# rdd0582/mri_superresolution

Hardware: AMD Instinct MI355X
Metric: 2D MRI slices/sec (train fwd+bwd) 256×256 U-Net; PSNR/SSIM vs ref (higher is better)
Workload: dtype bf16; 1 GPU; UNetSuperRes base_filters=64 depth=4, 256x256 slices -> 512x512, batch=16/GPU bf16, L1+SSIM(0.4), train step fwd+bwd+Adam+SSIM metric; global_batch=16, parallelism=dp1

## Files before the change

include/mrisr.h:

```cpp
#ifndef MRISR_H
#define MRISR_H

#include <stddef.h>
#include <stdint.h>

#ifdef __cplusplus
extern "C" {
#endif

#define MRISR_OK 0
#define MRISR_E_ARG (-1)
#define MRISR_E_SHAPE (-2)
#define MRISR_E_DTYPE (-3)
#define MRISR_E_HIP (-4)
#define MRISR_E_UNSUPPORTED (-5)

#define MRISR_F32 0
#define MRISR_BF16 1
#define MRISR_F16 2

#define MRISR_SRC_RAW 0
#define MRISR_SRC_NORM 1
#define MRISR_SRC_RELU 2
#define MRISR_SP_NONE 0
// ... 164 lines not shown
int mrisr_head_backward(int dtype, const void* x, const float* scale, const float* shift,
                        const float* w, const float* out, const float* dout, void* da, float* dw,
                        float* db, int N, int H, int W, int C, void* stream);
int mrisr_head_forward_multi(int dtype, const void* x, const float* scale, const float* shift,
                             const float* w, const float* b, float* out, int N, int H, int W, int C,
                             int K, void* stream);
int mrisr_head_backward_multi(int dtype, const void* x, const float* scale, const float* shift,
                              const float* w, const float* out, const float* dout, void* da,
                              float* dw, float* db, int N, int H, int W, int C, int K, void* stream);

int mrisr_ssim_l1_forward(const float* a, const float* b, double* sums, float* coef, int N, int H,
                          int W, float val_range, float sigma, void* stream);
int mrisr_ssim_l1_backward(const float* a, const float* b, const float* coef, const double* sums,
                           const float* gscale, float l1_w, float ssim_w, float* da, int N, int H,
                           int W, float sigma, void* stream);
int mrisr_ssim_l1_forward_win(const float* a, const float* b, double* sums, float* coef, int N, int H, int W,
                              float val_range, float sigma, int window_size, void* stream);
int mrisr_ssim_l1_backward_win(const float* a, const float* b, const float* coef, const double* sums,
                               const float* gscale, float l1_w, float ssim_w, float* da, int N, int H, int W,
                               float sigma, int window_size, void* stream);

int mrisr_loss_finalize(const double* sums, int N, int H, int W, float l1_w, float ssim_w, float* out,
                        void* stream);

int mrisr_image_metrics(const float* a, const float* b, double* sums, int N, int H, int W, float val_range, float sigma,
                        int window_size, void* stream);
int mrisr_metrics_finalize(const double* sums, int N, int H, int W, float val_range, double* out, void* stream);

int mrisr_vgg_input_channels(void);
int mrisr_vgg_input_forward(int dtype, const float* x, void* out, size_t npix, void* stream);
int mrisr_vgg_input_backward(int dtype, const void* dx3, const float* gscale, float scale, float* dimg,
                             size_t npix, void* stream);
int mrisr_maxpool2_forward(int dtype, const void* x, void* out, int N, int H, int W, int C, void* stream);
int mrisr_maxpool2_backward(int dtype, const void* x, const void* dy, void* dx, int N, int H, int W, int C,
                            int relu_gate, void* stream);
int mrisr_feature_loss(int dtype, const void* a, const void* b, size_t n, int kind, double* sum16, float* out,
                       void* da, int relu_gate, void* stream);

int mrisr_adam_step(float* p, const float* g, float* m, float* v, size_t n, float lr, float beta1,
                    float beta2, float eps, float weight_decay, int step, float grad_scale,
                    void* stream);
int mrisr_adam_step_amp(float* p, const float* g, float* m, float* v, size_t n, float lr, float beta1, float beta2,
                        float eps, float weight_decay, int* step_device, float grad_mul,
                        const float* loss_scale_device, const float* found_inf_device, void* stream);

int mrisr_u8_histogram(const uint8_t* img, size_t pixels_per_image, int batch, unsigned* hist, void* stream);
// ... 157 lines not shown
```

mri_superresolution_amd/_lib.py:

```python
from __future__ import annotations

import ctypes as C
import os

from .tuning import TUNING

_HERE = os.path.dirname(os.path.abspath(__file__))
LIB_PATH = TUNING.lib_path or os.path.join(_HERE, "libmrisr.so")

F32, BF16, F16 = 0, 1, 2
SRC_RAW, SRC_NORM, SRC_RELU = 0, 1, 2
SP_NONE, SP_POOL2, SP_UP2, SP_HEAD = 0, 1, 2, 3
COMBINE_CONCAT, COMBINE_BLEND = 0, 1
OUT_PLAIN, OUT_PIXEL_SHUFFLE2 = 0, 1
UP2_BILINEAR, UP2_BICUBIC, UP2_SHARP_BILINEAR = 0, 1, 2
WINDOW_F32, WINDOW_I16 = 0, 1
VOLBLEND_SET, VOLBLEND_ADD, VOLBLEND_FINISH = 0, 1, 2
MORPH_DILATE, MORPH_ERODE = 0, 1
RESAMPLE_LINEAR, RESAMPLE_CUBIC, RESAMPLE_AREA, RESAMPLE_LANCZOS4 = 1, 2, 3, 4
BIAS_PAIR, BIAS_HUM, BIAS_LOWPASS = 0, 1, 2
RESAMPLE_NEAREST = 5
PACK_RING = 256
PACK_UPADJ = 512
STAT_SLOTS = 16
# ... 79 lines not shown
    "mrisr_act_bwd_apply_fused": (_i, [_i, _vp, _fp, _fp, _i, C.POINTER(Consumer), _fp, _fp, C.POINTER(GnBwdFin), _vp, _i, _i,
                                       _i, _i, _vp]),
    "mrisr_act_bwd_onepass_slots": (_i, []),
    "mrisr_act_bwd_onepass_barrier_words": (_i, []),
    "mrisr_act_bwd_onepass_ok": (_i, [_i, _i, C.POINTER(Consumer), _i, _i, _i, _i]),
    "mrisr_act_bwd_onepass": (_i, [_i, _vp, _fp, _fp, _fp, _i, C.POINTER(Consumer), _fp, _vp, C.POINTER(GnBwdFin), _vp, _i, _i, _i,
                                   _i, _vp]),
    "mrisr_act_bwd_apply_fused_unshuffle": (_i, [_i, _vp, _fp, _fp, C.POINTER(Consumer), _fp, C.POINTER(GnBwdFin), _vp, _fp, _i,
                                                 _i, _i, _i, _vp]),
    "mrisr_act_bwd_blend_ok": (_i, [_i, _i, _i, _i, _i]),
    "mrisr_act_bwd_blend_reduce": (_i, [_i, _vp, C.POINTER(BlendBranch), C.POINTER(BlendBranch), _fp, _i, _i, _i, _i, _i, _vp]),
    "mrisr_act_bwd_blend_apply": (_i, [_i, _vp, C.POINTER(BlendBranch), C.POINTER(BlendBranch), _fp, C.POINTER(GnBwdFin),
                                       C.POINTER(GnBwdFin), _vp, _vp, _fp, _i, _i, _i, _i, _vp]),
    "mrisr_channel_sum": (_i, [_i, _vp, _fp, _sz, _i, _vp]),
    "mrisr_head_forward": (_i, [_i, _vp, _fp, _fp, _fp, _fp, _fp, _i, _i, _i, _i, _vp]),
    "mrisr_head_backward": (_i, [_i, _vp, _fp, _fp, _fp, _fp, _fp, _vp, _fp, _fp, _i, _i, _i, _i, _vp]),
    "mrisr_head_forward_multi": (_i, [_i, _vp, _fp, _fp, _fp, _fp, _fp, _i, _i, _i, _i, _i, _vp]),
    "mrisr_head_backward_multi": (_i, [_i, _vp, _fp, _fp, _fp, _fp, _fp, _vp, _fp, _fp, _i, _i, _i, _i, _i, _vp]),
    "mrisr_ssim_l1_forward": (_i, [_fp, _fp, _dp, _fp, _i, _i, _i, _f, _f, _vp]),
    "mrisr_ssim_l1_backward": (_i, [_fp, _fp, _fp, _dp, _fp, _f, _f, _fp, _i, _i, _i, _f, _vp]),
    "mrisr_ssim_l1_forward_win": (_i, [_fp, _fp, _dp, _fp, _i, _i, _i, _f, _f, _i, _vp]),
    "mrisr_ssim_l1_backward_win": (_i, [_fp, _fp, _fp, _dp, _fp, _f, _f, _fp, _i, _i, _i, _f, _i, _vp]),
    "mrisr_loss_finalize": (_i, [_dp, _i, _i, _i, _f, _f, _fp, _vp]),
    "mrisr_image_metrics": (_i, [_fp, _fp, _dp, _i, _i, _i, _f, _f, _i, _vp]),
    "mrisr_metrics_finalize": (_i, [_dp, _i, _i, _i, _f, _dp, _vp]),
    "mrisr_vgg_input_channels": (_i, []),
    "mrisr_vgg_input_forward": (_i, [_i, _fp, _vp, _sz, _vp]),
    "mrisr_vgg_input_backward": (_i, [_i, _vp, _fp, _f, _fp, _sz, _vp]),
    "mrisr_maxpool2_forward": (_i, [_i, _vp, _vp, _i, _i, _i, _i, _vp]),
    "mrisr_maxpool2_backward": (_i, [_i, _vp, _vp, _vp, _i, _i, _i, _i, _i, _vp]),
    "mrisr_feature_loss": (_i, [_i, _vp, _vp, _sz, _i, _dp, _fp, _vp, _i, _vp]),
    "mrisr_adam_step": (_i, [_fp, _fp, _fp, _fp, _sz, _f, _f, _f, _f, _f, _i, _f, _vp]),
    "mrisr_adam_step_amp": (_i, [_fp, _fp, _fp, _fp, _sz, _f, _f, _f, _f, _f, _vp, _f, _fp, _fp, _vp]),
    "mrisr_u8_histogram": (_i, [_vp, _sz, _i, _vp, _vp]),
    "mrisr_u8_percentile_normalise": (_i, [_vp, _vp, _sz, _i, _d, _d, _fp, _fp, _vp]),
    "mrisr_f32_to_u8": (_i, [_fp, _vp, _sz, _vp]),
    "mrisr_u8_upscale2": (_i, [_vp, _vp, _fp, _i, _i, _i, _i, _vp]),
    "mrisr_u8_to_unit_f32": (_i, [_vp, _fp, _sz, _vp]),
    "mrisr_augment_geo_u8": (_i, [_vp, _vp, _i, _i, _i, _vp, _dp, _vp]),
    "mrisr_augment_finish_u8": (_i, [_vp, _fp, _i, _sz, _vp, _dp, _vp]),
    "mrisr_lowfield_dirichlet": (_i, [_i, _d, _fp, _fp]),
    "mrisr_lowfield_workspace_bytes": (_sz, [_i, _i, _i]),
    "mrisr_lowfield_simulate": (_i, [_vp, _i, _i, _i, _d, _fp, _fp, _fp, _fp, _f, _fp, _fp, _vp, _vp, _vp, _fp, _vp]),
    "mrisr_lowfield_dirichlet_any": (_i, [_i, _d, _fp, _fp]),
    "mrisr_lowfield_simulate_f32": (_i, [_fp, _i, _i, _i, _d, _fp, _fp, _fp, _fp, _f, _fp, _fp, _vp, _vp, _fp, _vp]),
    "mrisr_resample_taps": (_i, [_i, _i, _i, _i, _vp, _vp, _fp]),
# ... 26 lines not shown
    "mrisr_f32_masked_percentiles_workspace_bytes": (_sz, [_i]),
    "mrisr_f32_volume_masked_percentiles": (_i, [_fp, _vp, _sz, C.POINTER(C.c_double), _i, _fp, _vp, _vp, _vp]),
    "mrisr_f32_volume_piecewise_map": (_i, [_fp, _sz, _fp, _fp, _i, _fp, _vp]),
    "mrisr_f32_volume_smooth_masked": (_i, [_fp, _vp, _vp, _i, _i, _i, _fp, _i, _fp, _i, _fp, _i, _fp, _fp, _fp, _vp]),
    "mrisr_f32_volume_bias_apply": (_i, [_fp, _sz, _fp, _fp, _fp, _fp, _fp, _vp, _f, _i, _fp, _fp, _vp]),
    "mrisr_f32_volume_nlm": (_i, [_fp, _i, _i, _i, _i, _i, _fp, _fp, _fp, _vp]),
    "mrisr_f32_volume_noise_workspace_bytes": (_sz, []),
    "mrisr_f32_volume_noise_params": (_i, [_fp, _vp, _sz, _f, _f, _fp, _vp, _vp, _vp]),
    "mrisr_f32_volume_deform_workspace_bytes": (_sz, []),
    "mrisr_f32_volume_warp": (_i, [_fp, _fp, _i, _i, _i, _i, _f, _fp, _vp]),
    "mrisr_f32_volume_demons_force": (_i, [_fp, _fp, _fp, _i, _i, _i, _f, _f, _fp, _vp, _vp, _vp]),
    "mrisr_f32_volume_field_smooth": (_i, [_fp, _fp, _i, _i, _i, _i, _fp, _i, _vp, _vp, _vp]),
    "mrisr_f32_volume_jacobian_stats": (_i, [_fp, _i, _i, _i, _fp, _vp, _vp, _vp]),
    "mrisr_f32_volume_field_compose": (_i, [_fp, _fp, _i, _i, _i, _fp, _vp]),
    "mrisr_f32_volume_demons_update": (_i, [_fp, _fp, _fp, _i, _i, _i, _f, _f, _f, _fp, _vp, _vp, _vp]),
    "mrisr_f32_volume_warp_matrix": (_i, [_fp, _i, _i, _i, _fp, _i, _i, _i, C.POINTER(C.c_double), _i, _f, _fp, _vp]),
    "mrisr_f32_volume_quantise": (_i, [_fp, _vp, _sz, _fp, _vp, _vp, _vp, _vp, _vp]),
    "mrisr_u8_volume_joint_hist": (_i, [_vp, _vp, _sz, _i, _vp, _vp]),
    "mrisr_u8_volume_icm_half": (_i, [_vp, _vp, _i, _i, _i, _i, _vp, _i, _i, _vp, _vp]),
    "mrisr_u8_volume_confusion": (_i, [_vp, _vp, _vp, _sz, _i, _vp, _vp]),
}

_lib = None
ABI_VERSION = 323


def load():
    global _lib
    if _lib is not None:
        return _lib
    if not os.path.exists(LIB_PATH):
        raise RuntimeError(
            f"{LIB_PATH} not found: the HIP kernel library is not built. Run "
            "`python -m mri_superresolution_amd.build` (needs hipcc); there is no CPU fallback.")
    lib = C.CDLL(LIB_PATH)
    missing = [name for name in SIGNATURES if not hasattr(lib, name)]
    if missing:
        raise RuntimeError(f"{LIB_PATH} lacks {len(missing)} symbol(s) of include/mrisr.h ({', '.join(missing[:4])}...): "
                           "header/library drift - rebuild with `python -m mri_superresolution_amd.build`")
    for name, (res, args) in SIGNATURES.items():
        fn = getattr(lib, name)
        fn.restype = res
        fn.argtypes = args
    if int(lib.mrisr_version()) != ABI_VERSION:
        raise RuntimeError(f"{LIB_PATH} is version {int(lib.mrisr_version())}, these bindings need {ABI_VERSION} (struct layouts "
                           "changed): rebuild with `python -m mri_superresolution_amd.build`")
    global STAT_SLOTS
# ... 48 lines not shown
```

mri_superresolution_amd/csrc/api.cpp:

```cpp
#include "common.h"
thread_local char g_mrisr_err[512] = "";
extern "C" const char* mrisr_last_error(void) { return g_mrisr_err; }
extern "C" int mrisr_version(void) { return 323; }
extern "C" int mrisr_stat_slots(void) { return MRISR_STAT_SLOTS; }
```

mri_superresolution_amd/csrc/loss.hip:

```cpp
#include "common.h"

constexpr int kMaxWin = 15;
constexpr int kTW = 32, kTH = 8;

struct GaussWin { float g[kMaxWin]; };

static GaussWin make_window(float sigma, int win) {
    GaussWin w;
    float sum = 0.f;
    for (int i = 0; i < kMaxWin; ++i) w.g[i] = 0.f;
    for (int i = 0; i < win; ++i) {
        const float c = (float)(i - win / 2);
        w.g[i] = expf(-(c * c) / (2.0f * sigma * sigma));
        sum += w.g[i];
    }
    for (int i = 0; i < win; ++i) w.g[i] /= sum;
    return w;
}

constexpr int kFT = 32;
template <int kWin, bool kSq = false>
__global__ __launch_bounds__(256) void ssim_l1_fwd_kernel(const float* __restrict__ a, const float* __restrict__ b,
                                                          double* __restrict__ sums, float* __restrict__ coef, int N,
                                                          int H, int W, float c1, float c2, const GaussWin win) {
    constexpr int kHalo = kWin / 2, kFL = kFT + 2 * kHalo;
    __shared__ float ta[kFL][kFL + 2], tb[kFL][kFL + 2];
    __shared__ float hz[5][kFL][kFT + 1];
    constexpr int kSums = kSq ? 3 : 2;
    __shared__ float part[4][kSums];
    const int t = threadIdx.x, n = blockIdx.z;
    const int x0 = blockIdx.x * kFT, y0 = blockIdx.y * kFT;
    const float* an = a + (size_t)n * H * W;
    const float* bn = b + (size_t)n * H * W;
    for (int i = t; i < kFL * kFL; i += 256) {
        const int ly = i / kFL, lx = i - ly * kFL;
        const int gy = y0 + ly - kHalo, gx = x0 + lx - kHalo;
        const bool in = gy >= 0 && gy < H && gx >= 0 && gx < W;
        ta[ly][lx] = in ? an[(size_t)gy * W + gx] : 0.f;
        tb[ly][lx] = in ? bn[(size_t)gy * W + gx] : 0.f;
    }
    __syncthreads();
    for (int sgm = t; sgm < kFL * (kFT / 4); sgm += 256) {
        const int ly = sgm / (kFT / 4), lx = (sgm - ly * (kFT / 4)) * 4;
        float u[kWin + 3], v[kWin + 3];
#pragma unroll
        for (int k = 0; k < kWin + 3; ++k) { u[k] = ta[ly][lx + k]; v[k] = tb[ly][lx + k]; }
#pragma unroll
        for (int o = 0; o < 4; ++o) {
            float s0 = 0.f, s1 = 0.f, s2 = 0.f, s3 = 0.f, s4 = 0.f;
#pragma unroll
            for (int k = 0; k < kWin; ++k) {
                const float uu = u[o + k], vv = v[o + k], g = win.g[k];
                s0 += g * uu; s1 += g * vv; s2 += g * uu * uu; s3 += g * vv * vv; s4 += g * uu * vv;
            }
            hz[0][ly][lx + o] = s0; hz[1][ly][lx + o] = s1; hz[2][ly][lx + o] = s2; hz[3][ly][lx + o] = s3; hz[4][ly][lx + o] = s4;
        }
    }
    __syncthreads();
    const int lx = t & (kFT - 1), ly0 = (t >> 5) * 4;
    float m[4][5];
#pragma unroll
    for (int o = 0; o < 4; ++o)
#pragma unroll
        for (int q = 0; q < 5; ++q) m[o][q] = 0.f;
#pragma unroll
    for (int q = 0; q < 5; ++q) {
        float col[kWin + 3];
#pragma unroll
        for (int k = 0; k < kWin + 3; ++k) col[k] = hz[q][ly0 + k][lx];
#pragma unroll
        for (int o = 0; o < 4; ++o)
#pragma unroll
            for (int k = 0; k < kWin; ++k) m[o][q] += win.g[k] * col[o + k];
    }
    float l1 = 0.f, sv = 0.f, sq = 0.f;
    const int gx = x0 + lx;
#pragma unroll
    for (int o = 0; o < 4; ++o) {
        const int gy = y0 + ly0 + o;
        if (gy < H && gx < W) {
            const float mu1 = m[o][0], mu2 = m[o][1];
            const float mu1sq = mu1 * mu1, mu2sq = mu2 * mu2, mu12 = mu1 * mu2;
            const float s11 = m[o][2] - mu1sq, s22 = m[o][3] - mu2sq, s12 = m[o][4] - mu12;
            const float A1 = 2.f * mu12 + c1, A2 = 2.f * s12 + c2, B1 = mu1sq + mu2sq + c1, B2 = s11 + s22 + c2;
            const float inv = 1.f / (B1 * B2);
            const float S = A1 * A2 * inv;
            sv += S;
            const float d = ta[ly0 + o + kHalo][lx + kHalo] - tb[ly0 + o + kHalo][lx + kHalo];
            l1 += fabsf(d);
            if (kSq) sq += d * d;
            if (coef) {
                const size_t plane = (size_t)N * H * W, oo = ((size_t)n * H + gy) * W + gx;
                coef[oo] = 2.f * mu2 * (A2 - A1) * inv - 2.f * mu1 * S / B1 + 2.f * mu1 * S / B2;
                coef[plane + oo] = -S / B2;
                coef[2 * plane + oo] = 2.f * A1 * inv;
            }
        }
    }
    l1 = wave_sum(l1);
    sv = wave_sum(sv);
    if (kSq) sq = wave_sum(sq);
    if ((t & 63) == 0) {
        part[t >> 6][0] = l1; part[t >> 6][1] = sv;
        if (kSq) part[t >> 6][kSums - 1] = sq;
    }
    __syncthreads();
    if (t < kSums) atomic_add_f64(&sums[(size_t)n * kSums + t], (double)(part[0][t] + part[1][t] + part[2][t] + part[3][t]));
}

template <int WIN>
static void launch_ssim_fwd(dim3 grid, hipStream_t s, const float* a, const float* b, double* sums, float* coef, int N, int H, int W,
                            float c1, float c2, float sigma) {
    ssim_l1_fwd_kernel<WIN><<<grid, 256, 0, s>>>(a, b, sums, coef, N, H, W, c1, c2, make_window(sigma, WIN));
}
#define MRISR_SSIM_WIN_SWITCH(win, CALL) \
    switch (win) { case 3: CALL(3); break; case 5: CALL(5); break; case 7: CALL(7); break; case 9: CALL(9); break; \
                   case 11: CALL(11); break; case 13: CALL(13); break; default: CALL(15); break; }

extern "C" int mrisr_ssim_l1_forward_win(const float* a, const float* b, double* sums, float* coef, int N, int H, int W,
                                         float val_range, float sigma, int window_size, void* stream) {
    if (!a || !b || !sums) MRISR_FAIL(MRISR_E_ARG, "ssim_l1_forward: null pointer");
    if (N <= 0 || H <= 0 || W <= 0 || N > 65535) MRISR_FAIL(MRISR_E_SHAPE, "ssim_l1_forward: N%d H%d W%d", N, H, W);
    if (window_size < 3 || window_size > kMaxWin || !(window_size & 1)) MRISR_FAIL(MRISR_E_UNSUPPORTED, "ssim_l1_forward: window_size %d (odd, 3..15)", window_size);
    const float c1 = (0.01f * val_range) * (0.01f * val_range), c2 = (0.03f * val_range) * (0.03f * val_range);
    dim3 grid(ceil_div(W, kFT), ceil_div(H, kFT), N);
    hipStream_t s = (hipStream_t)stream;
#define MRISR_CALL(WIN) launch_ssim_fwd<WIN>(grid, s, a, b, sums, coef, N, H, W, c1, c2, sigma)
    MRISR_SSIM_WIN_SWITCH(window_size, MRISR_CALL)
#undef MRISR_CALL
    MRISR_CHECK_LAUNCH("ssim_l1_forward");
    return MRISR_OK;
}
extern "C" int mrisr_ssim_l1_forward(const float* a, const float* b, double* sums, float* coef, int N, int H, int W,
                                     float val_range, float sigma, void* stream) {
    return mrisr_ssim_l1_forward_win(a, b, sums, coef, N, H, W, val_range, sigma, 11, stream);
}

template <int WIN>
static void launch_metrics(dim3 grid, hipStream_t s, const float* a, const float* b, double* sums, int N, int H, int W,
                           float c1, float c2, float sigma) {
    ssim_l1_fwd_kernel<WIN, true><<<grid, 256, 0, s>>>(a, b, sums, nullptr, N, H, W, c1, c2, make_window(sigma, WIN));
}
extern "C" int mrisr_image_metrics(const float* a, const float* b, double* sums, int N, int H, int W, float val_range,
                                   float sigma, int window_size, void* stream) {
    if (!a || !b || !sums) MRISR_FAIL(MRISR_E_ARG, "image_metrics: null pointer");
    if (N <= 0 || H <= 0 || W <= 0 || N > 65535) MRISR_FAIL(MRISR_E_SHAPE, "image_metrics: N%d H%d W%d", N, H, W);
    if (window_size < 3 || window_size > kMaxWin || !(window_size & 1)) MRISR_FAIL(MRISR_E_UNSUPPORTED, "image_metrics: window_size %d (odd, 3..15)", window_size);
    const float c1 = (0.01f * val_range) * (0.01f * val_range), c2 = (0.03f * val_range) * (0.03f * val_range);
    dim3 grid(ceil_div(W, kFT), ceil_div(H, kFT), N);
    hipStream_t s = (hipStream_t)stream;
#define MRISR_CALL(WIN) launch_metrics<WIN>(grid, s, a, b, sums, N, H, W, c1, c2, sigma)
    MRISR_SSIM_WIN_SWITCH(window_size, MRISR_CALL)
#undef MRISR_CALL
    MRISR_CHECK_LAUNCH("image_metrics");
    return MRISR_OK;
}

__global__ __launch_bounds__(64) void metrics_finalize_kernel(const double* __restrict__ sums, int N, double inv_pixels, double range2,
                                                              double* __restrict__ out) {
    const int n = blockIdx.x * 64 + threadIdx.x;
    if (n >= N) return;
    const double mae = sums[3 * n] * inv_pixels, ssim = sums[3 * n + 1] * inv_pixels, mse = sums[3 * n + 2] * inv_pixels;
    out[5 * n] = ssim;
    out[5 * n + 1] = mse;
    out[5 * n + 2] = __dsqrt_rn(mse);
    out[5 * n + 3] = mae;
    out[5 * n + 4] = mse < 1e-10 ? 100.0 : 10.0 * log10(range2 / mse);
}

extern "C" int mrisr_metrics_finalize(const double* sums, int N, int H, int W, float val_range, double* out, void* stream) {
    if (!sums || !out) MRISR_FAIL(MRISR_E_ARG, "metrics_finalize: null pointer");
    if (N <= 0 || H <= 0 || W <= 0) MRISR_FAIL(MRISR_E_SHAPE, "metrics_finalize: N%d H%d W%d", N, H, W);
    metrics_finalize_kernel<<<ceil_div(N, 64), 64, 0, (hipStream_t)stream>>>(sums, N, 1.0 / ((double)H * W), (double)val_range * (double)val_range, out);
    MRISR_CHECK_LAUNCH("metrics_finalize");
    return MRISR_OK;
}

template <int kWin>
__global__ __launch_bounds__(256) void ssim_l1_bwd_kernel(const float* __restrict__ a, const float* __restrict__ b,
                                                          const float* __restrict__ coef, const double* __restrict__ sums,
                                                          const float* __restrict__ gscale, float l1_w, float ssim_w,
                                                          float* __restrict__ da, int N, int H, int W, const GaussWin win) {
    constexpr int kHalo = kWin / 2, kLW = kTW + 2 * kHalo, kLH = kTH + 2 * kHalo;
    __shared__ float tc[3][kLH][kLW + 1];
    __shared__ float hz[3][kLH][kTW + 1];
    const int t = threadIdx.x, n = blockIdx.z;
    const int x0 = blockIdx.x * kTW, y0 = blockIdx.y * kTH;
    const size_t plane = (size_t)N * H * W;
    const float gs = gscale ? gscale[0] : 1.f;
    const double numel = (double)N * H * W;
    float sw = 0.f;
    if (ssim_w != 0.f) {
        if (sums) {
            double tot = 0.0;
            for (int i = 0; i < N; ++i) tot += sums[(size_t)i * 2 + 1];
            const double mean = tot / numel;
            if (mean >= 0.0 && mean <= 1.0) sw = ssim_w;
        } else {
            sw = ssim_w;
        }
    }
    if (sw != 0.f) {
        for (int i = t; i < kLH * kLW; i += 256) {
            const int ly = i / kLW, lx = i - ly * kLW;
            const int gy = y0 + ly - kHalo, gx = x0 + lx - kHalo;
            const bool in = gy >= 0 && gy < H && gx >= 0 && gx < W;
            const size_t o = ((size_t)n * H + gy) * W + gx;
#pragma unroll
            for (int q = 0; q < 3; ++q) tc[q][ly][lx] = in ? coef[q * plane + o] : 0.f;
        }
        __syncthreads();
        for (int i = t; i < kLH * kTW; i += 256) {
            const int ly = i / kTW, lx = i - ly * kTW;
            float s[3] = {0.f, 0.f, 0.f};
#pragma unroll
            for (int k = 0; k < kWin; ++k)
#pragma unroll
                for (int q = 0; q < 3; ++q) s[q] += win.g[k] * tc[q][ly][lx + k];
#pragma unroll
            for (int q = 0; q < 3; ++q) hz[q][ly][lx] = s[q];
        }
        __syncthreads();
    }
    const int ly = t / kTW, lx = t - ly * kTW;
    const int gy = y0 + ly, gx = x0 + lx;
    if (gy < H && gx < W) {
        const size_t o = ((size_t)n * H + gy) * W + gx;
        const float av = a[o], bv = b[o];
        float g = 0.f;
        if (l1_w != 0.f) {
            const float d = av - bv;
            g += l1_w * (d > 0.f ? 1.f : (d < 0.f ? -1.f : 0.f));
        }
        if (sw != 0.f) {
            float m[3] = {0.f, 0.f, 0.f};
#pragma unroll
            for (int k = 0; k < kWin; ++k)
#pragma unroll
                for (int q = 0; q < 3; ++q) m[q] += win.g[k] * hz[q][ly + k][lx];
            g -= sw * (m[0] + 2.f * av * m[1] + bv * m[2]);
        }
        da[o] = gs * g * (float)(1.0 / numel);
    }
}

template <int WIN>
static void launch_ssim_bwd(dim3 grid, hipStream_t s, const float* a, const float* b, const float* coef, const double* sums,
                            const float* gscale, float l1_w, float ssim_w, float* da, int N, int H, int W, float sigma) {
    ssim_l1_bwd_kernel<WIN><<<grid, 256, 0, s>>>(a, b, coef, sums, gscale, l1_w, ssim_w, da, N, H, W, make_window(sigma, WIN));
}
extern "C" int mrisr_ssim_l1_backward_win(const float* a, const float* b, const float* coef, const double* sums,
                                          const float* gscale, float l1_w, float ssim_w, float* da, int N, int H, int W,
                                          float sigma, int window_size, void* stream) {
    if (!a || !b || !da) MRISR_FAIL(MRISR_E_ARG, "ssim_l1_backward: null pointer");
    if (ssim_w != 0.f && !coef) MRISR_FAIL(MRISR_E_ARG, "ssim_l1_backward: ssim term needs coef");
    if (N <= 0 || H <= 0 || W <= 0 || N > 65535) MRISR_FAIL(MRISR_E_SHAPE, "ssim_l1_backward: N%d H%d W%d", N, H, W);
    if (window_size < 3 || window_size > kMaxWin || !(window_size & 1)) MRISR_FAIL(MRISR_E_UNSUPPORTED, "ssim_l1_backward: window_size %d (odd, 3..15)", window_size);
    dim3 grid(ceil_div(W, kTW), ceil_div(H, kTH), N);
    hipStream_t s = (hipStream_t)stream;
#define MRISR_CALL(WIN) launch_ssim_bwd<WIN>(grid, s, a, b, coef, sums, gscale, l1_w, ssim_w, da, N, H, W, sigma)
    MRISR_SSIM_WIN_SWITCH(window_size, MRISR_CALL)
#undef MRISR_CALL
    MRISR_CHECK_LAUNCH("ssim_l1_backward");
    return MRISR_OK;
}
extern "C" int mrisr_ssim_l1_backward(const float* a, const float* b, const float* coef, const double* sums,
                                      const float* gscale, float l1_w, float ssim_w, float* da, int N, int H, int W,
                                      float sigma, void* stream) {
    return mrisr_ssim_l1_backward_win(a, b, coef, sums, gscale, l1_w, ssim_w, da, N, H, W, sigma, 11, stream);
}

__global__ void loss_finalize_kernel(const double* __restrict__ sums, int N, double inv_numel, double inv_per_sample,
                                     float l1_w, float ssim_w, float* __restrict__ out) {
    if (threadIdx.x != 0 || blockIdx.x != 0) return;
    double l1 = 0.0, ss = 0.0;
    for (int i = 0; i < N; ++i) {
        l1 += sums[2 * i];
        ss += sums[2 * i + 1];
        out[3 + i] = (float)(sums[2 * i + 1] * inv_per_sample);
    }
    const float l1m = (float)(l1 * inv_numel), sm = (float)(ss * inv_numel);
    float total = 0.f;
    if (l1_w > 0.f) total += l1_w * l1m;
    if (ssim_w > 0.f) total += ssim_w * (1.f - fminf(fmaxf(sm, 0.f), 1.f));
    out[0] = total;
    out[1] = l1m;
    out[2] = sm;
}

extern "C" int mrisr_loss_finalize(const double* sums, int N, int H, int W, float l1_w, float ssim_w, float* out,
                                   void* stream) {
    if (!sums || !out) MRISR_FAIL(MRISR_E_ARG, "loss_finalize: null pointer");
    loss_finalize_kernel<<<1, 64, 0, (hipStream_t)stream>>>(sums, N, 1.0 / ((double)N * H * W), 1.0 / ((double)H * W), l1_w, ssim_w, out);
    MRISR_CHECK_LAUNCH("loss_finalize");
    return MRISR_OK;
}
```

mri_superresolution_amd/utils/losses.py:

```python
from __future__ import annotations

import torch
import torch.nn as nn

from .. import _lib as L

VGG_MEAN = [0.485, 0.456, 0.406]
VGG_STD = [0.229, 0.224, 0.225]

_WINDOW = 11


def gaussian_window(window_size: int, sigma: float):
    coords = torch.arange(window_size, dtype=torch.float32) - window_size // 2
    g = torch.exp(-(coords ** 2) / (2 * sigma ** 2))
    return g / g.sum()


def create_window(window_size: int, channel: int, sigma: float, device: torch.device):
    w1 = gaussian_window(window_size, sigma).to(device).unsqueeze(1)
    return w1.mm(w1.t()).expand(channel, 1, window_size, window_size).contiguous()


def _planes(t: torch.Tensor) -> torch.Tensor:
# ... 11 lines not shown
def _sums_key(a, b, sigma, val_range, win):
    return (a.data_ptr(), a._version, tuple(a.shape), b.data_ptr(), b._version, float(sigma), float(val_range), int(win),
            L.inplace_epoch, torch.cuda.current_stream().cuda_stream)


def _check_window(window_size):
    if not isinstance(window_size, int) or window_size < 3 or window_size > 15 or window_size % 2 == 0:
        raise NotImplementedError(f"the fused SSIM kernel supports odd window sizes 3..15, got {window_size!r}")


class _SSIML1(torch.autograd.Function):

    @staticmethod
    def forward(ctx, img1, img2, l1_w, ssim_w, sigma, val_range, kind, holder, track, win=_WINDOW, track2=False):
        a, b = _planes(img1), _planes(img2)
        if a.shape != b.shape:
            raise ValueError(f"shape mismatch {tuple(a.shape)} vs {tuple(b.shape)}")
        n, c, h, w = a.shape
        planes = n * c
        need_grad = bool(track)
        st = L.stream_ptr()
        global _last_sums
        key = _sums_key(a, b, sigma, val_range, win)
        if not need_grad and not track2 and _last_sums is not None and _last_sums[0] == key:
            sums, coef = _last_sums[1], None
        else:
            sums = torch.zeros(planes * 2, dtype=torch.float64, device=a.device)
            coef = torch.empty(3 * planes * h * w, dtype=torch.float32, device=a.device) if (need_grad and ssim_w != 0) else None
            L.call("mrisr_ssim_l1_forward_win", a.data_ptr(), b.data_ptr(), sums.data_ptr(), L.ptr(coef), planes, h, w,
                   float(val_range), float(sigma), int(win), st, nbytes=planes * h * w * (8 + (12 if coef is not None else 0)))
            _last_sums = (key, sums, a, b)
        comp = torch.empty(3 + planes, dtype=torch.float32, device=a.device)
        L.call("mrisr_loss_finalize", sums.data_ptr(), planes, h, w, float(l1_w), float(ssim_w), comp.data_ptr(), st)
        if holder is not None:
            holder.last_components = comp
        ctx.save_for_backward(a, b, coef, sums)
        ctx.cfg = (float(l1_w), float(ssim_w), float(sigma), kind, planes, h, w, int(win), float(val_range), bool(track), bool(track2))
        return comp[0].clone() if kind == 0 else comp[2].clone()

    @staticmethod
    def backward(ctx, gout):
        a, b, coef, sums = ctx.saved_tensors
        l1_w, ssim_w, sigma, kind, planes, h, w, win, val_range, track, track2 = ctx.cfg
        g = gout.detach().to(torch.float32).reshape(1).contiguous()
        st = L.stream_ptr()

        def grad_first(x, y, cf):
            dx = torch.empty_like(x)
            if kind == 0:
                L.call("mrisr_ssim_l1_backward_win", x.data_ptr(), y.data_ptr(), L.ptr(cf), sums.data_ptr(), g.data_ptr(),
                       l1_w, ssim_w, dx.data_ptr(), planes, h, w, sigma, win, st,
                       nbytes=planes * h * w * (12 + (12 if cf is not None else 0)))
            else:
                L.call("mrisr_ssim_l1_backward_win", x.data_ptr(), y.data_ptr(), L.ptr(cf), None, g.data_ptr(),
                       0.0, -1.0, dx.data_ptr(), planes, h, w, sigma, win, st)
            return dx

        da = grad_first(a, b, coef) if track else None
        db = None
        if track2:
            coef2 = None
            if ssim_w != 0:
                coef2 = torch.empty(3 * planes * h * w, dtype=torch.float32, device=a.device)
                scratch = torch.zeros(planes * 2, dtype=torch.float64, device=a.device)
                L.call("mrisr_ssim_l1_forward_win", b.data_ptr(), a.data_ptr(), scratch.data_ptr(), coef2.data_ptr(), planes, h, w,
                       val_range, sigma, win, st)
            db = grad_first(b, a, coef2)
        return da, db, None, None, None, None, None, None, None, None, None


def ssim(img1, img2, window_size=11, sigma=1.5, val_range=1.0, device=None, window=None, size_average=True):
    _check_window(window_size)
    holder = type("H", (), {})()
    grads = torch.is_grad_enabled()
    val = _SSIML1.apply(img1, img2, 0.0, 1.0, sigma, val_range, 1, holder, grads and img1.requires_grad, window_size,
                        grads and img2.requires_grad)
    if size_average:
        result = val
    else:
        n, c = img1.shape[0], img1.shape[1]
        result = holder.last_components[3:].view(n, c).mean(1)
    if img1.dtype != torch.float32 and img1.dtype == img2.dtype:
        result = result.to(img1.dtype)
    return result


class VGGFeatureExtractor(nn.Module):

# ... 112 lines not shown
```

Measured before the change: 2113 slices/s.

## Restructure SSIM+L1 loss kernels: vectorized tile loads, per-tile slots, fused finalize

The SSIM/L1 forward kernel now loads its halo tile with float4 pieces into registers before writing shared memory. Each block writes its partial sums to a per-tile slot instead of doing a double atomicAdd, and a single finalize kernel reduces the slots and writes the scalar return value. This removes the zero-fill memset, the float64 atomics and the clone kernel. The backward kernel moves to the same 32x32 tiles with 4 outputs per thread, vectorized coef loads and a wave-parallel gate reduction. The SSIM loss is a small part of a full U-Net train step, and the change adds slot buffer allocations and more shared memory per block.

Measured after the change: 2128 slices/s (median of 6 runs). No clear change (+0.7%).

```diff
diff --git a/include/mrisr.h b/include/mrisr.h
--- a/include/mrisr.h
+++ b/include/mrisr.h
@@ -210,6 +210,11 @@
 
 int mrisr_loss_finalize(const double* sums, int N, int H, int W, float l1_w, float ssim_w, float* out,
                         void* stream);
+int mrisr_ssim_l1_tiles(int H, int W);
+int mrisr_ssim_l1_forward_slots(const float* a, const float* b, double* slots, float* coef, int N, int H, int W,
+                                float val_range, float sigma, int window_size, void* stream);
+int mrisr_loss_finalize_slots(const double* slots, double* sums, int N, int H, int W, float l1_w, float ssim_w, float* out,
+                              float* ret, int kind, void* stream);
 
 int mrisr_image_metrics(const float* a, const float* b, double* sums, int N, int H, int W, float val_range, float sigma,
                         int window_size, void* stream);
diff --git a/mri_superresolution_amd/_lib.py b/mri_superresolution_amd/_lib.py
--- a/mri_superresolution_amd/_lib.py
+++ b/mri_superresolution_amd/_lib.py
@@ -125,6 +125,9 @@
     "mrisr_ssim_l1_forward_win": (_i, [_fp, _fp, _dp, _fp, _i, _i, _i, _f, _f, _i, _vp]),
     "mrisr_ssim_l1_backward_win": (_i, [_fp, _fp, _fp, _dp, _fp, _f, _f, _fp, _i, _i, _i, _f, _i, _vp]),
     "mrisr_loss_finalize": (_i, [_dp, _i, _i, _i, _f, _f, _fp, _vp]),
+    "mrisr_ssim_l1_tiles": (_i, [_i, _i]),
+    "mrisr_ssim_l1_forward_slots": (_i, [_fp, _fp, _dp, _fp, _i, _i, _i, _f, _f, _i, _vp]),
+    "mrisr_loss_finalize_slots": (_i, [_dp, _dp, _i, _i, _i, _f, _f, _fp, _fp, _i, _vp]),
     "mrisr_image_metrics": (_i, [_fp, _fp, _dp, _i, _i, _i, _f, _f, _i, _vp]),
     "mrisr_metrics_finalize": (_i, [_dp, _i, _i, _i, _f, _dp, _vp]),
     "mrisr_vgg_input_channels": (_i, []),
@@ -197,7 +200,7 @@
 }
 
 _lib = None
-ABI_VERSION = 323
+ABI_VERSION = 324
 
 
 def load():
diff --git a/mri_superresolution_amd/csrc/api.cpp b/mri_superresolution_amd/csrc/api.cpp
--- a/mri_superresolution_amd/csrc/api.cpp
+++ b/mri_superresolution_amd/csrc/api.cpp
@@ -1,5 +1,5 @@
 #include "common.h"
 thread_local char g_mrisr_err[512] = "";
 extern "C" const char* mrisr_last_error(void) { return g_mrisr_err; }
-extern "C" int mrisr_version(void) { return 323; }
+extern "C" int mrisr_version(void) { return 324; }
 extern "C" int mrisr_stat_slots(void) { return MRISR_STAT_SLOTS; }
diff --git a/mri_superresolution_amd/csrc/loss.hip b/mri_superresolution_amd/csrc/loss.hip
--- a/mri_superresolution_amd/csrc/loss.hip
+++ b/mri_superresolution_amd/csrc/loss.hip
@@ -1,7 +1,6 @@
 #include "common.h"
 
 constexpr int kMaxWin = 15;
-constexpr int kTW = 32, kTH = 8;
 
 struct GaussWin { float g[kMaxWin]; };
 
@@ -19,42 +18,94 @@
 }
 
 constexpr int kFT = 32;
+constexpr int kApron = 8;
+constexpr int kSW = kFT + 2 * kApron;
+constexpr int kSS = kSW + 1;
+constexpr int kHS = kFT + 1;
+
+static inline int ssim_tiles(int H, int W) { return ceil_div(W, kFT) * ceil_div(H, kFT); }
+
+__device__ __forceinline__ float4 load_piece(const float* __restrict__ p, int gy, int gx, int H, int W, bool vec) {
+    const bool row_in = gy >= 0 && gy < H;
+    const float* row = p + (size_t)min(max(gy, 0), H - 1) * W;
+    float4 v;
+    if (vec) {
+        v = *reinterpret_cast<const float4*>(row + min(max(gx, 0), W - 4));
+        if (!(row_in && gx >= 0 && gx < W)) v = make_float4(0.f, 0.f, 0.f, 0.f);
+    } else {
+        v.x = row[min(max(gx, 0), W - 1)];
+        v.y = row[min(max(gx + 1, 0), W - 1)];
+        v.z = row[min(max(gx + 2, 0), W - 1)];
+        v.w = row[min(max(gx + 3, 0), W - 1)];
+        if (!(row_in && gx >= 0 && gx < W)) v.x = 0.f;
+        if (!(row_in && gx + 1 >= 0 && gx + 1 < W)) v.y = 0.f;
+        if (!(row_in && gx + 2 >= 0 && gx + 2 < W)) v.z = 0.f;
+        if (!(row_in && gx + 3 >= 0 && gx + 3 < W)) v.w = 0.f;
+    }
+    return v;
+}
+__device__ __forceinline__ void store_piece(float* __restrict__ row, float4 v) {
+    row[0] = v.x; row[1] = v.y; row[2] = v.z; row[3] = v.w;
+}
+#define MRISR_PIECE(i, ly, lc)            \
+    const int pq_ = (i) / (kSW / 4);      \
+    const int lc = ((i) - pq_ * (kSW / 4)) * 4, ly = min(pq_, kFL - 1)
+
+template <int kWin, int kOut, int kPlane>
+__device__ __forceinline__ void ssim_fwd_hblur(const float* __restrict__ pa, const float* __restrict__ pb, float* __restrict__ ph,
+                                               const GaussWin& win) {
+    float u[kWin + kOut - 1], v[kWin + kOut - 1];
+#pragma unroll
+    for (int k = 0; k < kWin + kOut - 1; ++k) { u[k] = pa[k]; v[k] = pb[k]; }
+#pragma unroll
+    for (int o = 0; o < kOut; ++o) {
+        float s0 = 0.f, s1 = 0.f, s2 = 0.f, s3 = 0.f, s4 = 0.f;
+#pragma unroll
+        for (int k = 0; k < kWin; ++k) {
+            const float uu = u[o + k], vv = v[o + k], g = win.g[k];
+            s0 += g * uu; s1 += g * vv; s2 += g * uu * uu; s3 += g * vv * vv; s4 += g * uu * vv;
+        }
+        ph[o] = s0; ph[kPlane + o] = s1; ph[2 * kPlane + o] = s2; ph[3 * kPlane + o] = s3; ph[4 * kPlane + o] = s4;
+    }
+}
+
 template <int kWin, bool kSq = false>
 __global__ __launch_bounds__(256) void ssim_l1_fwd_kernel(const float* __restrict__ a, const float* __restrict__ b,
-                                                          double* __restrict__ sums, float* __restrict__ coef, int N,
-                                                          int H, int W, float c1, float c2, const GaussWin win) {
+                                                          double* __restrict__ sums, double* __restrict__ slots,
+                                                          float* __restrict__ coef, int N, int H, int W, float c1, float c2,
+                                                          const GaussWin win) {
     constexpr int kHalo = kWin / 2, kFL = kFT + 2 * kHalo;
-    __shared__ float ta[kFL][kFL + 2], tb[kFL][kFL + 2];
-    __shared__ float hz[5][kFL][kFT + 1];
+    constexpr int kOff = kApron - kHalo;
+    constexpr int kPieces = kFL * (kSW / 4), kRounds = (kPieces + 255) / 256;
+    __shared__ float ta[kFL][kSS], tb[kFL][kSS];
+    __shared__ float hz[5][kFL][kHS];
     constexpr int kSums = kSq ? 3 : 2;
     __shared__ float part[4][kSums];
     const int t = threadIdx.x, n = blockIdx.z;
     const int x0 = blockIdx.x * kFT, y0 = blockIdx.y * kFT;
     const float* an = a + (size_t)n * H * W;
     const float* bn = b + (size_t)n * H * W;
-    for (int i = t; i < kFL * kFL; i += 256) {
-        const int ly = i / kFL, lx = i - ly * kFL;
-        const int gy = y0 + ly - kHalo, gx = x0 + lx - kHalo;
-        const bool in = gy >= 0 && gy < H && gx >= 0 && gx < W;
-        ta[ly][lx] = in ? an[(size_t)gy * W + gx] : 0.f;
-        tb[ly][lx] = in ? bn[(size_t)gy * W + gx] : 0.f;
+    const bool vec = (W & 3) == 0 && (((uintptr_t)a | (uintptr_t)b) & 15) == 0;
+    float4 ra[kRounds], rb[kRounds];
+#pragma unroll
+    for (int r = 0; r < kRounds; ++r) {
+        MRISR_PIECE(t + r * 256, ly, lc);
+        ra[r] = load_piece(an, y0 + ly - kHalo, x0 - kApron + lc, H, W, vec);
+        rb[r] = load_piece(bn, y0 + ly - kHalo, x0 - kApron + lc, H, W, vec);
+    }
+#pragma unroll
+    for (int r = 0; r < kRounds; ++r) {
+        MRISR_PIECE(t + r * 256, ly, lc);
+        if (t + r * 256 < kPieces) { store_piece(&ta[ly][lc], ra[r]); store_piece(&tb[ly][lc], rb[r]); }
     }
     __syncthreads();
-    for (int sgm = t; sgm < kFL * (kFT / 4); sgm += 256) {
-        const int ly = sgm / (kFT / 4), lx = (sgm - ly * (kFT / 4)) * 4;
-        float u[kWin + 3], v[kWin + 3];
-#pragma unroll
-        for (int k = 0; k < kWin + 3; ++k) { u[k] = ta[ly][lx + k]; v[k] = tb[ly][lx + k]; }
-#pragma unroll
-        for (int o = 0; o < 4; ++o) {
-            float s0 = 0.f, s1 = 0.f, s2 = 0.f, s3 = 0.f, s4 = 0.f;
-#pragma unroll
-            for (int k = 0; k < kWin; ++k) {
-                const float uu = u[o + k], vv = v[o + k], g = win.g[k];
-                s0 += g * uu; s1 += g * vv; s2 += g * uu * uu; s3 += g * vv * vv; s4 += g * uu * vv;
-            }
-            hz[0][ly][lx + o] = s0; hz[1][ly][lx + o] = s1; hz[2][ly][lx + o] = s2; hz[3][ly][lx + o] = s3; hz[4][ly][lx + o] = s4;
-        }
+    {
+        const int ly = t >> 3, lx = (t & 7) * 4;
+        ssim_fwd_hblur<kWin, 4, kFL * kHS>(&ta[ly][lx + kOff], &tb[ly][lx + kOff], &hz[0][ly][lx], win);
+    }
+    if (t < (kFL - 32) * (kFT / 2)) {
+        const int ly = 32 + (t >> 4), lx = (t & 15) * 2;
+        ssim_fwd_hblur<kWin, 2, kFL * kHS>(&ta[ly][lx + kOff], &tb[ly][lx + kOff], &hz[0][ly][lx], win);
     }
     __syncthreads();
     const int lx = t & (kFT - 1), ly0 = (t >> 5) * 4;
@@ -86,7 +137,7 @@
             const float inv = 1.f / (B1 * B2);
             const float S = A1 * A2 * inv;
             sv += S;
-            const float d = ta[ly0 + o + kHalo][lx + kHalo] - tb[ly0 + o + kHalo][lx + kHalo];
+            const float d = ta[ly0 + o + kHalo][lx + kApron] - tb[ly0 + o + kHalo][lx + kApron];
             l1 += fabsf(d);
             if (kSq) sq += d * d;
             if (coef) {
@@ -105,41 +156,58 @@
         if (kSq) part[t >> 6][kSums - 1] = sq;
     }
     __syncthreads();
-    if (t < kSums) atomic_add_f64(&sums[(size_t)n * kSums + t], (double)(part[0][t] + part[1][t] + part[2][t] + part[3][t]));
+    if (t < kSums) {
+        const double v = (double)(part[0][t] + part[1][t] + part[2][t] + part[3][t]);
+        if (slots) {
+            const size_t tile = (size_t)blockIdx.y * gridDim.x + blockIdx.x, tiles = (size_t)gridDim.x * gridDim.y;
+            slots[((size_t)n * tiles + tile) * kSums + t] = v;
+        } else {
+            atomic_add_f64(&sums[(size_t)n * kSums + t], v);
+        }
+    }
 }
 
 template <int WIN>
-static void launch_ssim_fwd(dim3 grid, hipStream_t s, const float* a, const float* b, double* sums, float* coef, int N, int H, int W,
-                            float c1, float c2, float sigma) {
-    ssim_l1_fwd_kernel<WIN><<<grid, 256, 0, s>>>(a, b, sums, coef, N, H, W, c1, c2, make_window(sigma, WIN));
+static void launch_ssim_fwd(dim3 grid, hipStream_t s, const float* a, const float* b, double* sums, double* slots, float* coef, int N,
+                            int H, int W, float c1, float c2, float sigma) {
+    ssim_l1_fwd_kernel<WIN><<<grid, 256, 0, s>>>(a, b, sums, slots, coef, N, H, W, c1, c2, make_window(sigma, WIN));
 }
 #define MRISR_SSIM_WIN_SWITCH(win, CALL) \
     switch (win) { case 3: CALL(3); break; case 5: CALL(5); break; case 7: CALL(7); break; case 9: CALL(9); break; \
                    case 11: CALL(11); break; case 13: CALL(13); break; default: CALL(15); break; }
 
-extern "C" int mrisr_ssim_l1_forward_win(const float* a, const float* b, double* sums, float* coef, int N, int H, int W,
-                                         float val_range, float sigma, int window_size, void* stream) {
-    if (!a || !b || !sums) MRISR_FAIL(MRISR_E_ARG, "ssim_l1_forward: null pointer");
+static int ssim_l1_forward(const float* a, const float* b, double* sums, double* slots, float* coef, int N, int H, int W,
+                           float val_range, float sigma, int window_size, void* stream) {
+    if (!a || !b || (!sums && !slots)) MRISR_FAIL(MRISR_E_ARG, "ssim_l1_forward: null pointer");
     if (N <= 0 || H <= 0 || W <= 0 || N > 65535) MRISR_FAIL(MRISR_E_SHAPE, "ssim_l1_forward: N%d H%d W%d", N, H, W);
     if (window_size < 3 || window_size > kMaxWin || !(window_size & 1)) MRISR_FAIL(MRISR_E_UNSUPPORTED, "ssim_l1_forward: window_size %d (odd, 3..15)", window_size);
     const float c1 = (0.01f * val_range) * (0.01f * val_range), c2 = (0.03f * val_range) * (0.03f * val_range);
     dim3 grid(ceil_div(W, kFT), ceil_div(H, kFT), N);
     hipStream_t s = (hipStream_t)stream;
-#define MRISR_CALL(WIN) launch_ssim_fwd<WIN>(grid, s, a, b, sums, coef, N, H, W, c1, c2, sigma)
+#define MRISR_CALL(WIN) launch_ssim_fwd<WIN>(grid, s, a, b, sums, slots, coef, N, H, W, c1, c2, sigma)
     MRISR_SSIM_WIN_SWITCH(window_size, MRISR_CALL)
 #undef MRISR_CALL
     MRISR_CHECK_LAUNCH("ssim_l1_forward");
     return MRISR_OK;
 }
+extern "C" int mrisr_ssim_l1_forward_win(const float* a, const float* b, double* sums, float* coef, int N, int H, int W,
+                                         float val_range, float sigma, int window_size, void* stream) {
+    return ssim_l1_forward(a, b, sums, nullptr, coef, N, H, W, val_range, sigma, window_size, stream);
+}
 extern "C" int mrisr_ssim_l1_forward(const float* a, const float* b, double* sums, float* coef, int N, int H, int W,
                                      float val_range, float sigma, void* stream) {
     return mrisr_ssim_l1_forward_win(a, b, sums, coef, N, H, W, val_range, sigma, 11, stream);
 }
+extern "C" int mrisr_ssim_l1_tiles(int H, int W) { return H > 0 && W > 0 ? ssim_tiles(H, W) : 0; }
+extern "C" int mrisr_ssim_l1_forward_slots(const float* a, const float* b, double* slots, float* coef, int N, int H, int W,
+                                           float val_range, float sigma, int window_size, void* stream) {
+    return ssim_l1_forward(a, b, nullptr, slots, coef, N, H, W, val_range, sigma, window_size, stream);
+}
 
 template <int WIN>
 static void launch_metrics(dim3 grid, hipStream_t s, const float* a, const float* b, double* sums, int N, int H, int W,
                            float c1, float c2, float sigma) {
-    ssim_l1_fwd_kernel<WIN, true><<<grid, 256, 0, s>>>(a, b, sums, nullptr, N, H, W, c1, c2, make_window(sigma, WIN));
+    ssim_l1_fwd_kernel<WIN, true><<<grid, 256, 0, s>>>(a, b, sums, nullptr, nullptr, N, H, W, c1, c2, make_window(sigma, WIN));
 }
 extern "C" int mrisr_image_metrics(const float* a, const float* b, double* sums, int N, int H, int W, float val_range,
                                    float sigma, int window_size, void* stream) {
@@ -176,71 +244,121 @@
     return MRISR_OK;
 }
 
+template <int kWin, int kOut, int kSrc, int kPlane>
+__device__ __forceinline__ void ssim_bwd_hblur(const float* __restrict__ pc, float* __restrict__ ph, const GaussWin& win) {
+#pragma unroll
+    for (int q = 0; q < 3; ++q) {
+        float u[kWin + kOut - 1];
+#pragma unroll
+        for (int k = 0; k < kWin + kOut - 1; ++k) u[k] = pc[q * kSrc + k];
+#pragma unroll
+        for (int o = 0; o < kOut; ++o) {
+            float s = 0.f;
+#pragma unroll
+            for (int k = 0; k < kWin; ++k) s += win.g[k] * u[o + k];
+            ph[q * kPlane + o] = s;
+        }
+    }
+}
+
 template <int kWin>
 __global__ __launch_bounds__(256) void ssim_l1_bwd_kernel(const float* __restrict__ a, const float* __restrict__ b,
                                                           const float* __restrict__ coef, const double* __restrict__ sums,
                                                           const float* __restrict__ gscale, float l1_w, float ssim_w,
                                                           float* __restrict__ da, int N, int H, int W, const GaussWin win) {
-    constexpr int kHalo = kWin / 2, kLW = kTW + 2 * kHalo, kLH = kTH + 2 * kHalo;
-    __shared__ float tc[3][kLH][kLW + 1];
-    __shared__ float hz[3][kLH][kTW + 1];
+    constexpr int kHalo = kWin / 2, kFL = kFT + 2 * kHalo, kOff = kApron - kHalo;
+    constexpr int kPieces = kFL * (kSW / 4), kRounds = (kPieces + 255) / 256;
+    __shared__ float tc[3][kFL][kSS];
+    __shared__ float hz[3][kFL][kHS];
+    __shared__ float gate;
     const int t = threadIdx.x, n = blockIdx.z;
-    const int x0 = blockIdx.x * kTW, y0 = blockIdx.y * kTH;
+    const int x0 = blockIdx.x * kFT, y0 = blockIdx.y * kFT;
     const size_t plane = (size_t)N * H * W;
+    const double numel = (double)N * H * W;
+    const bool use_ssim = ssim_w != 0.f;
+    float4 rc[3][kRounds];
+    if (use_ssim) {
+        const bool vec = (W & 3) == 0 && ((uintptr_t)coef & 15) == 0;
+#pragma unroll
+        for (int r = 0; r < kRounds; ++r) {
+            MRISR_PIECE(t + r * 256, ly, lc);
+#pragma unroll
+            for (int q = 0; q < 3; ++q)
+                rc[q][r] = load_piece(coef + q * plane + (size_t)n * H * W, y0 + ly - kHalo, x0 - kApron + lc, H, W, vec);
+        }
+    }
+    const int lx = t & (kFT - 1), ly0 = (t >> 5) * 4;
+    const int gx = x0 + lx;
+    float av[4], bv[4];
+#pragma unroll
+    for (int o = 0; o < 4; ++o) {
+        const size_t oc = ((size_t)n * H + min(y0 + ly0 + o, H - 1)) * W + min(gx, W - 1);
+        av[o] = a[oc]; bv[o] = b[oc];
+    }
     const float gs = gscale ? gscale[0] : 1.f;
-    const double numel = (double)N * H * W;
-    float sw = 0.f;
-    if (ssim_w != 0.f) {
-        if (sums) {
-            double tot = 0.0;
-            for (int i = 0; i < N; ++i) tot += sums[(size_t)i * 2 + 1];
-            const double mean = tot / numel;
-            if (mean >= 0.0 && mean <= 1.0) sw = ssim_w;
-        } else {
-            sw = ssim_w;
-        }
-    }
+    if (t < 64) {
+        float open = 0.f;
+        if (use_ssim) {
+            if (sums) {
+                double tot = 0.0;
+                for (int i = t; i < N; i += 64) tot += sums[(size_t)i * 2 + 1];
+                const double mean = wave_sum_d(tot) / numel;
+                if (mean >= 0.0 && mean <= 1.0) open = ssim_w;
+            } else {
+                open = ssim_w;
+            }
+        }
+        if (t == 0) gate = open;
+    }
+    __syncthreads();
+    const float sw = gate;
+    float m[4][3];
+#pragma unroll
+    for (int o = 0; o < 4; ++o)
+#pragma unroll
+        for (int q = 0; q < 3; ++q) m[o][q] = 0.f;
     if (sw != 0.f) {
-        for (int i = t; i < kLH * kLW; i += 256) {
-            const int ly = i / kLW, lx = i - ly * kLW;
-            const int gy = y0 + ly - kHalo, gx = x0 + lx - kHalo;
-            const bool in = gy >= 0 && gy < H && gx >= 0 && gx < W;
-            const size_t o = ((size_t)n * H + gy) * W + gx;
-#pragma unroll
-            for (int q = 0; q < 3; ++q) tc[q][ly][lx] = in ? coef[q * plane + o] : 0.f;
+#pragma unroll
+        for (int r = 0; r < kRounds; ++r) {
+            MRISR_PIECE(t + r * 256, ly, lc);
+            if (t + r * 256 < kPieces) {
+#pragma unroll
+                for (int q = 0; q < 3; ++q) store_piece(&tc[q][ly][lc], rc[q][r]);
+            }
         }
         __syncthreads();
-        for (int i = t; i < kLH * kTW; i += 256) {
-            const int ly = i / kTW, lx = i - ly * kTW;
-            float s[3] = {0.f, 0.f, 0.f};
-#pragma unroll
-            for (int k = 0; k < kWin; ++k)
-#pragma unroll
-                for (int q = 0; q < 3; ++q) s[q] += win.g[k] * tc[q][ly][lx + k];
-#pragma unroll
-            for (int q = 0; q < 3; ++q) hz[q][ly][lx] = s[q];
+        {
+            const int ly = t >> 3, sx = (t & 7) * 4;
+            ssim_bwd_hblur<kWin, 4, kFL * kSS, kFL * kHS>(&tc[0][ly][sx + kOff], &hz[0][ly][sx], win);
+        }
+        if (t < (kFL - 32) * (kFT / 2)) {
+            const int ly = 32 + (t >> 4), sx = (t & 15) * 2;
+            ssim_bwd_hblur<kWin, 2, kFL * kSS, kFL * kHS>(&tc[0][ly][sx + kOff], &hz[0][ly][sx], win);
         }
         __syncthreads();
-    }
-    const int ly = t / kTW, lx = t - ly * kTW;
-    const int gy = y0 + ly, gx = x0 + lx;
-    if (gy < H && gx < W) {
-        const size_t o = ((size_t)n * H + gy) * W + gx;
-        const float av = a[o], bv = b[o];
-        float g = 0.f;
-        if (l1_w != 0.f) {
-            const float d = av - bv;
-            g += l1_w * (d > 0.f ? 1.f : (d < 0.f ? -1.f : 0.f));
-        }
-        if (sw != 0.f) {
-            float m[3] = {0.f, 0.f, 0.f};
-#pragma unroll
-            for (int k = 0; k < kWin; ++k)
-#pragma unroll
-                for (int q = 0; q < 3; ++q) m[q] += win.g[k] * hz[q][ly + k][lx];
-            g -= sw * (m[0] + 2.f * av * m[1] + bv * m[2]);
-        }
-        da[o] = gs * g * (float)(1.0 / numel);
+#pragma unroll
+        for (int q = 0; q < 3; ++q) {
+            float col[kWin + 3];
+#pragma unroll
+            for (int k = 0; k < kWin + 3; ++k) col[k] = hz[q][ly0 + k][lx];
+#pragma unroll
+            for (int o = 0; o < 4; ++o)
+#pragma unroll
+                for (int k = 0; k < kWin; ++k) m[o][q] += win.g[k] * col[o + k];
+        }
+    }
+#pragma unroll
+    for (int o = 0; o < 4; ++o) {
+        const int gy = y0 + ly0 + o;
+        if (gy < H && gx < W) {
+            float g = 0.f;
+            if (l1_w != 0.f) {
+                const float d = av[o] - bv[o];
+                g += l1_w * (d > 0.f ? 1.f : (d < 0.f ? -1.f : 0.f));
+            }
+            if (sw != 0.f) g -= sw * (m[o][0] + 2.f * av[o] * m[o][1] + bv[o] * m[o][2]);
+            da[((size_t)n * H + gy) * W + gx] = gs * g * (float)(1.0 / numel);
+        }
     }
 }
 
@@ -256,7 +374,7 @@
     if (ssim_w != 0.f && !coef) MRISR_FAIL(MRISR_E_ARG, "ssim_l1_backward: ssim term needs coef");
     if (N <= 0 || H <= 0 || W <= 0 || N > 65535) MRISR_FAIL(MRISR_E_SHAPE, "ssim_l1_backward: N%d H%d W%d", N, H, W);
     if (window_size < 3 || window_size > kMaxWin || !(window_size & 1)) MRISR_FAIL(MRISR_E_UNSUPPORTED, "ssim_l1_backward: window_size %d (odd, 3..15)", window_size);
-    dim3 grid(ceil_div(W, kTW), ceil_div(H, kTH), N);
+    dim3 grid(ceil_div(W, kFT), ceil_div(H, kFT), N);
     hipStream_t s = (hipStream_t)stream;
 #define MRISR_CALL(WIN) launch_ssim_bwd<WIN>(grid, s, a, b, coef, sums, gscale, l1_w, ssim_w, da, N, H, W, sigma)
     MRISR_SSIM_WIN_SWITCH(window_size, MRISR_CALL)
@@ -295,3 +413,45 @@
     MRISR_CHECK_LAUNCH("loss_finalize");
     return MRISR_OK;
 }
+
+__global__ __launch_bounds__(1024) void loss_finalize_slots_kernel(const double* __restrict__ slots, int tiles, double* sums, int N,
+                                                                   double inv_numel, double inv_per_sample, float l1_w, float ssim_w,
+                                                                   float* __restrict__ out, float* __restrict__ ret, int kind) {
+    const int t = threadIdx.x;
+    if (slots) {
+        for (int p = t >> 6; p < 2 * N; p += 16) {
+            const double* sp = slots + (size_t)(p >> 1) * tiles * 2 + (p & 1);
+            double s = 0.0;
+            for (int i = t & 63; i < tiles; i += 64) s += sp[(size_t)i * 2];
+            s = wave_sum_d(s);
+            if ((t & 63) == 0) sums[p] = s;
+        }
+        __syncthreads();
+    }
+    if (t != 0) return;
+    double l1 = 0.0, ss = 0.0;
+    for (int i = 0; i < N; ++i) {
+        l1 += sums[2 * i];
+        ss += sums[2 * i + 1];
+        out[3 + i] = (float)(sums[2 * i + 1] * inv_per_sample);
+    }
+    const float l1m = (float)(l1 * inv_numel), sm = (float)(ss * inv_numel);
+    float total = 0.f;
+    if (l1_w > 0.f) total += l1_w * l1m;
+    if (ssim_w > 0.f) total += ssim_w * (1.f - fminf(fmaxf(sm, 0.f), 1.f));
+    out[0] = total;
+    out[1] = l1m;
+    out[2] = sm;
+    if (ret) ret[0] = kind == 0 ? total : sm;
+}
+
+extern "C" int mrisr_loss_finalize_slots(const double* slots, double* sums, int N, int H, int W, float l1_w, float ssim_w,
+                                         float* out, float* ret, int kind, void* stream) {
+    if (!sums || !out) MRISR_FAIL(MRISR_E_ARG, "loss_finalize_slots: null pointer");
+    if (N <= 0 || H <= 0 || W <= 0 || N > 65535) MRISR_FAIL(MRISR_E_SHAPE, "loss_finalize_slots: N%d H%d W%d", N, H, W);
+    if (kind != 0 && kind != 1) MRISR_FAIL(MRISR_E_ARG, "loss_finalize_slots: kind %d (0 total, 1 ssim)", kind);
+    loss_finalize_slots_kernel<<<1, 1024, 0, (hipStream_t)stream>>>(slots, ssim_tiles(H, W), sums, N, 1.0 / ((double)N * H * W),
+                                                                    1.0 / ((double)H * W), l1_w, ssim_w, out, ret, kind);
+    MRISR_CHECK_LAUNCH("loss_finalize_slots");
+    return MRISR_OK;
+}
diff --git a/mri_superresolution_amd/utils/losses.py b/mri_superresolution_amd/utils/losses.py
--- a/mri_superresolution_amd/utils/losses.py
+++ b/mri_superresolution_amd/utils/losses.py
@@ -57,21 +57,31 @@
         st = L.stream_ptr()
         global _last_sums
         key = _sums_key(a, b, sigma, val_range, win)
-        if not need_grad and not track2 and _last_sums is not None and _last_sums[0] == key:
-            sums, coef = _last_sums[1], None
+        hit = not need_grad and not track2 and _last_sums is not None and _last_sums[0] == key
+        if hit and kind == 1:
+            sums, coef, comp = _last_sums[1], None, _last_sums[4]
+            ret = comp[2]
         else:
-            sums = torch.zeros(planes * 2, dtype=torch.float64, device=a.device)
-            coef = torch.empty(3 * planes * h * w, dtype=torch.float32, device=a.device) if (need_grad and ssim_w != 0) else None
-            L.call("mrisr_ssim_l1_forward_win", a.data_ptr(), b.data_ptr(), sums.data_ptr(), L.ptr(coef), planes, h, w,
-                   float(val_range), float(sigma), int(win), st, nbytes=planes * h * w * (8 + (12 if coef is not None else 0)))
-            _last_sums = (key, sums, a, b)
-        comp = torch.empty(3 + planes, dtype=torch.float32, device=a.device)
-        L.call("mrisr_loss_finalize", sums.data_ptr(), planes, h, w, float(l1_w), float(ssim_w), comp.data_ptr(), st)
+            comp = torch.empty(3 + planes, dtype=torch.float32, device=a.device)
+            ret = torch.empty((), dtype=torch.float32, device=a.device)
+            if hit:
+                sums, coef, slots = _last_sums[1], None, None
+            else:
+                tiles = L.load().mrisr_ssim_l1_tiles(h, w)
+                slots = torch.empty(planes * tiles * 2, dtype=torch.float64, device=a.device)
+                sums = torch.empty(planes * 2, dtype=torch.float64, device=a.device)
+                coef = torch.empty(3 * planes * h * w, dtype=torch.float32, device=a.device) if (need_grad and ssim_w != 0) else None
+                L.call("mrisr_ssim_l1_forward_slots", a.data_ptr(), b.data_ptr(), slots.data_ptr(), L.ptr(coef), planes, h, w,
+                       float(val_range), float(sigma), int(win), st, nbytes=planes * h * w * (8 + (12 if coef is not None else 0)))
+            L.call("mrisr_loss_finalize_slots", L.ptr(slots), sums.data_ptr(), planes, h, w, float(l1_w), float(ssim_w),
+                   comp.data_ptr(), ret.data_ptr(), int(kind), st)
+            if not hit:
+                _last_sums = (key, sums, a, b, comp)
         if holder is not None:
             holder.last_components = comp
         ctx.save_for_backward(a, b, coef, sums)
         ctx.cfg = (float(l1_w), float(ssim_w), float(sigma), kind, planes, h, w, int(win), float(val_range), bool(track), bool(track2))
-        return comp[0].clone() if kind == 0 else comp[2].clone()
+        return ret
 
     @staticmethod
     def backward(ctx, gout):
@@ -97,8 +107,8 @@
             coef2 = None
             if ssim_w != 0:
                 coef2 = torch.empty(3 * planes * h * w, dtype=torch.float32, device=a.device)
-                scratch = torch.zeros(planes * 2, dtype=torch.float64, device=a.device)
-                L.call("mrisr_ssim_l1_forward_win", b.data_ptr(), a.data_ptr(), scratch.data_ptr(), coef2.data_ptr(), planes, h, w,
+                scratch = torch.empty(planes * L.load().mrisr_ssim_l1_tiles(h, w) * 2, dtype=torch.float64, device=a.device)
+                L.call("mrisr_ssim_l1_forward_slots", b.data_ptr(), a.data_ptr(), scratch.data_ptr(), coef2.data_ptr(), planes, h, w,
                        val_range, sigma, win, st)
             db = grad_first(b, a, coef2)
         return da, db, None, None, None, None, None, None, None, None, None
```
